# ToyotaResearchInstitute/conex

Measured on AMD Instinct MI355X. Metric: Newton KKT-solves/sec (assemble+factor+solve), 1000x(20x20) PSD blocks, fp64, higher is better.
Workload: dtype f64

## Files before the change

conex_amd/csrc/kkt_context.hip:

```cpp
#include <hip/hip_ext.h>
#include "kkt_internal.h"
#include "kernels_cone.hip.h"
#include "kernels_gemm.hip.h"
#include "kernels_kkt_big.hip.h"
#include "kernels_oct.hip.h"
#include "kernels_lmi.hip.h"
#include "lmi_fused_mfma.h"
#include "kernels_lmi_sparse.hip.h"
#include "kernels_lmi_rows.hip.h"
#include "kernels_lmi_large.hip.h"
#include "kernels_quad.hip.h"


namespace cxk_host {

int Fail(cxk_context* ctx, const char* msg) {
  ctx->err = msg;
  fprintf(stderr, "conex_kkt_hip: %s\n", msg);
  return CXK_FAILURE;
}

bool IsUnique(int N, int m, const int* x) {
  std::vector<char> seen(N > 0 ? N : 1, 0);
  for (int i = 0; i < m; i++) {
// ... 879 lines not shown
    const size_t lds = sizeof(double) * 65 * ((NA_) > (NB_) ? (NA_) : (NB_)) + sizeof(SnRec) * (size_t)std::min(nchain, kChainRing); \
    if (mode == 0)                                                                                          \
      tree_chain_lean<0, NA_, SA_, NB_, SB_><<<1, 64, lds, ctx->stream>>>(                                  \
          ctx->plan, ctx->p_rec.p, pos0, nchain, ctx->slab.p, ctx->y.p, ctx->d_fail.p, RhsIn{});            \
    else                                                                                                    \
      tree_chain_lean<1, NA_, SA_, NB_, SB_><<<1, 64, lds, ctx->stream>>>(                                  \
          ctx->plan, ctx->p_rec.p, pos0, nchain, ctx->slab.p, ctx->y.p, ctx->d_fail.p, ctx->rhs_in);        \
  }
    CXK_CHAIN(8, 8, 8, 8)
    CXK_CHAIN(16, 8, 16, 8)
    CXK_CHAIN(24, 0, 24, 0)
    CXK_CHAIN(24, 8, 24, 8)
    CXK_CHAIN(32, 16, 32, 16)
    CXK_CHAIN(8, 8, 24, 0)
    CXK_CHAIN(16, 8, 24, 0)
    CXK_CHAIN(8, 8, 16, 8)
    CXK_CHAIN(24, 0, 24, 8)
    CXK_CHAIN(24, 0, 32, 16)
#undef CXK_CHAIN
    CXK_DEMAND(done, "internal error: no tree_chain_lean instance for the chain's shapes");
    CXK_TRY(hipGetLastError());
  return CXK_SUCCESS;
}

int MakeFusedTreeArgs(cxk_context* ctx, FusedTreeArgs* out) {
  if (*ctx->fx_flag != 0.0) {
    CXK_TRY(hipStreamSynchronize(ctx->stream));
    CXK_TRY(hipMemcpy(ctx->fx_hand.p, ctx->fx_hand_init.data(), sizeof(double) * ctx->fx_hand_init.size(), hipMemcpyHostToDevice));
    unsigned long long bits = kFusedSentinel;
    double sent;
    memcpy(&sent, &bits, sizeof(sent));
    std::vector<double> ys(ctx->fx_ysig.n, sent);
    CXK_TRY(hipMemcpy(ctx->fx_ysig.p, ys.data(), sizeof(double) * ys.size(), hipMemcpyHostToDevice));
    if (ctx->fx_done.p) {
      CXK_TRY(hipMemset(ctx->fx_done.p, 0, sizeof(unsigned long long) * ctx->fx_done.n));
      ctx->fx_done_target = 0;
    }
    *ctx->fx_flag = 0.0;
    ctx->timeout_pending = true;
  }
  FusedTreeArgs& a = *out;
  a.rec = ctx->fx_rec.p;
  a.count = (int)ctx->level_sn.size();
  a.G = ctx->G.p;
  a.AWc = ctx->AWc.p;
  a.AQcc = ctx->AQcc.p;
  a.b = ctx->b.p;
  a.AW = ctx->AW.p;
  a.AQc = ctx->AQc.p;
  a.slab = ctx->slab.p;
  a.y = ctx->y.p;
  a.pub = ctx->fx_pub.p;
  a.tg_reg = ctx->tg_reg.p;
  a.xreg = ctx->fx_xreg.p;
  a.xsrc = ctx->fx_xsrc.p;
  a.rsrc = ctx->fx_rsrc.p;
  a.hand = ctx->fx_hand.p;
  a.hand_stride = (long long)(ctx->fx_hand.n / 2);
  a.updb_base = ctx->fx_updb_base;
  a.ysig = ctx->fx_ysig.p;
  a.ysig_stride = (long long)(ctx->fx_ysig.n / 2);
  a.gen = (int)(ctx->fused_gen++ & 1u);
  a.tgen = (int)(ctx->fused_tgen & 1u);
  a.fwd_stride = ctx->fx_fwd_stride;
  a.y_stride = ctx->md.N;
  a.y3 = ctx->y3.p;
  a.fail = ctx->d_fail.p;
  a.tag = ctx->fail_tag;
  a.k = a.bs = a.cs = a.cb = a.cq = a.cw = 0;
  a.k_from = nullptr;
  a.comb = 0;
  a.form = 0;
  a.sc = ctx->sc.p;
  a.sys_sc = ctx->sys_sc.p;
  a.K = (int)ctx->cons.size();
  a.host_flag = ctx->fx_flag;
  a.up_sleep = 30;
  a.count_up = ctx->fused_shard ? ctx->fused_up : a.count;
  a.x = ctx->xbuf.p;
  a.n_xs = ctx->n_xs;
  a.n_xv = ctx->n_xv;
  a.xg = ctx->fx_xg.p;
  a.as_src = ctx->as_src.p;
  a.xs_pt = ctx->xs_pt.p;
  a.pt_ptr = ctx->pt_ptr.p;
  a.pt_src = ctx->pt_src.p;
  a.xr = ctx->fx_xr.p;
  a.rs_src = ctx->rs_src.p;
  a.pf_ptr = ctx->pf_ptr.p;
  a.pf_src = ctx->pf_src.p;
  a.done = ctx->fx_done.p;
  a.done_target = 0;
  return CXK_SUCCESS;
}

int ShardAllReduce(cxk_context* ctx, double* buf, size_t count, int op);
// ... 28 lines not shown
  a.done_target = ++ctx->fx_done_target;
  const bool hook = ctx->debug_timeout_at >= 0 && ctx->fused_launches++ == ctx->debug_timeout_at;
  CXK_TRY(LaunchFusedTree(a, ctx->fused_sa, ctx->fused_sb, kFusedShardUp, ctx->stream));
  if (hook && ctx->debug_timeout_site == CXK_DEBUG_FUSED_SHARD_UP && DebugReportTimeout(ctx)) return CXK_FAILURE;
  if (*ctx->fx_flag != 0.0) {
    static const double kTimedOut[2] = {1.0, 1.0};
    CXK_TRY(hipMemcpyAsync(ctx->xbuf.p + ExchangeCount(ctx) - 2, kTimedOut, sizeof(kTimedOut), hipMemcpyHostToDevice,
                           ctx->stream));
  }
  if (ShardAllReduce(ctx, ctx->xbuf.p, (size_t)ExchangeCount(ctx), 0 )) return CXK_FAILURE;
  ctx->shard_fused_tag = ctx->asm_tag;
  ctx->shard_launch_collectives = ctx->collectives;
  CXK_TRY(LaunchFusedTree(a, ctx->fused_sa, ctx->fused_sb, kFusedShardTop, ctx->stream));
  if (hook && ctx->debug_timeout_site == CXK_DEBUG_FUSED_SHARD_TOP && DebugReportTimeout(ctx)) return CXK_FAILURE;
  return CXK_SUCCESS;
}

int LaunchFusedTreeSolve(cxk_context* ctx) {
  const cxk_context::AsmPending ap = ctx->asm_pending;
  ctx->asm_pending.on = false;
  FusedTreeArgs a;
  if (MakeFusedTreeArgs(ctx, &a)) return CXK_FAILURE;
  ctx->asm_tag = ctx->asm_tag >= (1 << 30) ? 1 : ctx->asm_tag + 1;
  a.tag = ctx->fail_tag = ctx->asm_tag;
  a.k = ap.k;
  a.bs = ap.bs;
  a.cs = ap.cs;
  a.cb = ap.cb;
  a.cq = ap.cq;
  a.cw = ap.cw;
  a.comb = ap.with_rhs == 2;
  if (ap.with_rhs == 3) {
    ctx->fused_tgen++;
    CXK_TRY(LaunchFusedTree(a, ctx->fused_sa, ctx->fused_sb, kFusedTriple, ctx->stream, ctx->clk_e0, ctx->clk_e1));
  } else if (ctx->fused_split) {
    CXK_TRY(LaunchFusedTree(a, ctx->fused_sa, ctx->fused_sb, kFusedUp, ctx->stream));
    CXK_TRY(LaunchFusedTree(a, ctx->fused_sa, ctx->fused_sb, kFusedDown, ctx->stream));
  } else {
    CXK_TRY(LaunchFusedTree(a, ctx->fused_sa, ctx->fused_sb, kFusedFull, ctx->stream, ctx->clk_e0, ctx->clk_e1));
  }
  if (ctx->debug_timeout_at >= 0 && ctx->fused_launches++ == ctx->debug_timeout_at &&
      ctx->debug_timeout_site == CXK_DEBUG_FUSED_FACTOR && DebugReportTimeout(ctx))
    return CXK_FAILURE;
  return CXK_SUCCESS;
}

int LaunchFusedTreeSweep(cxk_context* ctx) {
  FusedTreeArgs a;
  if (MakeFusedTreeArgs(ctx, &a)) return CXK_FAILURE;
  const RhsIn& ri = ctx->rhs_in;
  a.form = ri.form;
  a.k = ri.k;
  a.k_from = ri.k_from;
  a.bs = ri.bs;
  a.cs = ri.cs;
  a.cb = ri.cb;
  a.cq = ri.cq;
  a.cw = ri.cw;
  if (ctx->fused_split) {
    CXK_TRY(LaunchFusedTree(a, ctx->fused_sa, ctx->fused_sb, kFusedForward, ctx->stream));
    CXK_TRY(LaunchFusedTree(a, ctx->fused_sa, ctx->fused_sb, kFusedDown, ctx->stream));
  } else {
    CXK_TRY(LaunchFusedTree(a, ctx->fused_sa, ctx->fused_sb, kFusedSolve, ctx->stream, ctx->clk_e0, ctx->clk_e1));
  }
  return CXK_SUCCESS;
}

bool FusedTimedOut(const cxk_context* ctx) { return ctx->timeout_pending || (ctx->fx_flag && *ctx->fx_flag != 0.0); }

int DisableFusedTree(cxk_context* ctx) {
  CXK_TRY(hipStreamSynchronize(ctx->stream));
// ... 2350 lines not shown
```

conex_amd/csrc/kkt_internal.h:

```cpp
#pragma once
#include <hip/hip_runtime.h>
#include <dlfcn.h>
#include <rccl/rccl.h>

#include <algorithm>
#include <atomic>
#include <cfloat>
#include <climits>
#include <cmath>
#include <cstdio>
#include <cstdlib>
#include <cstring>
#include <iterator>
#include <map>
#include <memory>
#include <string>
#include <tuple>
#include <vector>

#include "../../include/conex_kkt_hip.h"
#include "kernels_kkt.hip.h"
#include "kernels_kkt_top.hip.h"
#include "lmi_types.h"
#include "symbolic.h"
// ... 157 lines not shown
  DevBuf<SnRec> p_rec;
  DevBuf<int> pub_dst, pubb_dst;
  DevBuf<double> upd, updb, xbuf;
  DevBuf<int64_t> xs_off, pt_dst, pt_src;
  DevBuf<int> xv_idx, pt_ptr, pf_ptr, pf_src, xs_pt;
  int64_t as_T = 0;
  bool fused_asm = false;
  DevBuf<AsmRec> asm_rec;
  DevBuf<GatherRec> as_rec2;
  DevBuf<ResidRec> rs_rec2;
  DevBuf<int> rs_var2;
  int64_t as_T2 = 0;
  int rs_N2 = 0;
  struct AsmPending {
    bool on = false;
    int with_rhs = 0;
    double k = 0, bs = 0, cs = 0, cb = 0, cq = 0, cw = 0;
  } asm_pending;
  bool fused_tree = false;
  bool fused_split = false;
  bool fused_sweep = false;
  bool fused_shard = false;
  int fused_up = 0;
  DevBuf<GatherRec> fx_xg;
  DevBuf<ResidRec> fx_xr;
  DevBuf<unsigned long long> fx_done;
  unsigned long long fx_done_target = 0;
  int fused_sa = 0, fused_sb = 0;
  DevBuf<int> fx_rec, fx_xreg;
  DevBuf<long long> fx_xsrc, fx_rsrc;
  DevBuf<int> fx_pub;
  DevBuf<double> fx_hand, fx_ysig;
  std::vector<double> fx_hand_init;
  long long fx_updb_base = 0;
  long long fx_fwd_stride = 0;
  unsigned fused_tgen = 0;
  DevBuf<double> y3;
  bool y3_valid = false;
  double y3_bs = 0, y3_cs = 0;
  bool y_deferred = false;
  bool no_y_deferral = false;
  DevBuf<unsigned long long> y_done;
  unsigned long long y_done_target = 0;
  bool no_triple = false;
  unsigned fused_gen = 0;
  double* fx_flag = nullptr;
  int debug_timeout_at = -1, debug_timeout_site = 0, fused_launches = 0;
  int fused_timeouts = 0;
  bool timeout_pending = false;
  bool timeout_unreported = false;
  long long shard_settled_seq = -1;
  int shard_fused_tag = 0;
  long long collectives = 0, shard_launch_collectives = 0;
  bool debug_stream_ordered = false;
  long long calls = 0, redo_call = -1;
  bool asm_deferred = false;
  bool forward_all_lean = false;
  RhsIn rhs_in{};
  int asm_tag = 0;
  bool fail_clean = false;
  int fail_tag = 0;
  FactorPlan plan{};
  unsigned long long lanczos_calls = 0;
  int dual_start = -1;
  bool use_ldlt = false;
  DevBuf<int> d_tr, d_reg;
// ... 84 lines not shown
```

conex_amd/csrc/kkt_plans.hip:

```cpp
#define CXK_DEVICE_FUNCTIONS_ONLY
#include "kkt_internal.h"
#include "big_chol.h"

namespace cxk_host {

void ComputeTreeStructure(cxk_context* ctx) {
  const Layout& L = ctx->lay;
  const int K = ctx->md.K;
  ctx->t_ns.assign(K, 0);
  ctx->t_nsep.assign(K, 0);
  ctx->t_start.assign(K, 0);
  ctx->t_level.assign(K, 0);
  ctx->t_parent.assign(K, -1);
  for (int e = 0; e < K; e++) {
    ctx->t_ns[e] = L.supernode_size[e];
    ctx->t_nsep[e] = (int)L.separators[e].size();
    ctx->t_start[e] = L.supernode_start[e];
    if (ctx->t_nsep[e] > 0) ctx->t_parent[e] = L.var_to_sn[L.separators[e][0]];
  }
  for (int i = 0; i < K; i++) {
    if (ctx->t_ns[i] == 0) continue;
    for (int v : L.separators[i]) {
      const int p = L.var_to_sn[v];
      if (ctx->t_level[p] < ctx->t_level[i] + 1) ctx->t_level[p] = ctx->t_level[i] + 1;
    }
  }
  ctx->nlev = 0;
  for (int e = 0; e < K; e++)
    if (ctx->t_ns[e] > 0) ctx->nlev = std::max(ctx->nlev, ctx->t_level[e] + 1);
}

double ConstraintWork(const ConstraintRec& c) {
  const double n = c.n, m = c.m;
// ... 84 lines not shown
      ctx->sn_mine[e] = 1;
      ctx->owned[i] = (rr++ % G) == ctx->rank;
    } else {
      const bool mine = owner_of_root[root_of[e]] == ctx->rank;
      ctx->sn_mine[e] = mine;
      ctx->owned[i] = mine;
    }
  }
  for (int p = 0; p < ctx->md.N; p++) ctx->var_valid[p] = ctx->sn_mine[ctx->lay.var_to_sn[p]];
  for (int e = 0; e < K; e++)
    if (ctx->sn_top[e]) {
      const int64_t n = ctx->t_ns[e];
      ctx->n_xs += n * (n + 1) / 2 + n * ctx->t_nsep[e];
      ctx->n_xv += (int)n;
    }
}

namespace {

struct PlanSwitches {
  bool no_big_dataflow = getenv("CXK_NO_BIG_DATAFLOW") != nullptr;
  bool debug_levels = getenv("CXK_DEBUG_LEVELS") != nullptr;
  bool no_lean = getenv("CXK_NO_LEAN") != nullptr;
  bool no_ranges = getenv("CXK_NO_RANGES") != nullptr;
  bool keep_top = getenv("CXK_KEEP_TOP") != nullptr;
  bool no_chain = getenv("CXK_NO_CHAIN") != nullptr;
  bool no_back_pairs = getenv("CXK_NO_BACK_PAIRS") != nullptr;
  bool no_fused_asm = getenv("CXK_NO_FUSED_ASM") != nullptr;
  bool no_fused_shard = getenv("CXK_NO_FUSED_SHARD") != nullptr;
  bool no_fused_tree = getenv("CXK_NO_FUSED_TREE") != nullptr;
  bool no_fused_wide = getenv("CXK_NO_FUSED_WIDE") != nullptr;
  bool fused_split = getenv("CXK_FUSED_SPLIT") != nullptr;
  bool fused_level_order = getenv("CXK_FUSED_LEVEL_ORDER") != nullptr;
  bool no_fused_sweep = getenv("CXK_NO_FUSED_SWEEP") != nullptr;
  bool no_top_dense = getenv("CXK_NO_TOP_DENSE") != nullptr;
};

struct Verdict {
  bool ok = true;
  const char* why = nullptr;
  bool check(bool cond, const char* msg) {
    ok = ok && cond;
    if (!ok && !why) why = msg;
    return ok;
  }
  void note(const char* msg) { check(true, msg); }
  int refuse(const PlanSwitches& sw, const char* strategy) const {
    if (sw.debug_levels) fprintf(stderr, "%s not taken: %s\n", strategy, why ? why : "(unnamed check)");
    return CXK_SUCCESS;
  }
};

template <typename Rec>
std::vector<Rec> Flatten(const std::vector<std::vector<int64_t>>& lists, std::vector<int>* ptr, std::vector<int64_t>* src) {
  std::vector<Rec> recs(lists.size());
  ptr->assign(lists.size() + 1, 0);
  for (size_t t = 0; t < lists.size(); t++) {
    for (int64_t q : lists[t]) src->push_back(q);
    (*ptr)[t + 1] = (int)src->size();
    const int len = (*ptr)[t + 1] - (*ptr)[t];
    recs[t].first = len > 0 ? (*src)[(*ptr)[t]] : -1;
    recs[t].beg = (*ptr)[t] + 1;
    recs[t].extra = len > 0 ? len - 1 : 0;
  }
  return recs;
}
// ... 695 lines not shown
      ok = rg.per[pvar].size() == 1 && rg.per[pvar][0] == ar.r_off + r[a];
      var_own[pvar] = 1;
    }
  }
  v.check(ok, "a level-0 supernode that is not a leaf with single sources in its own constraint's block");
  if (!v.ok) return v.refuse(sw, "fused assembly");
  std::vector<GatherRec> g2;
  for (size_t t = 0; t < ag.rec.size(); t++)
    if (!slab_own[t]) g2.push_back(ag.rec[t]);
  std::vector<ResidRec> r2;
  std::vector<int> v2;
  for (int pvar = 0; pvar < N; pvar++)
    if (!var_own[pvar]) {
      r2.push_back(rg.rec[pvar]);
      v2.push_back(pvar);
    }
  ctx->as_T2 = (int64_t)g2.size();
  ctx->rs_N2 = (int)v2.size();
  if (g2.empty()) g2.push_back(GatherRec{0, -1, 0, 0});
  if (v2.empty()) {
    r2.push_back(ResidRec{-1, 0, 0});
    v2.push_back(0);
  }
  CXK_TRY(ctx->asm_rec.upload(arecs));
  CXK_TRY(ctx->as_rec2.upload(g2));
  CXK_TRY(ctx->rs_rec2.upload(r2));
  CXK_TRY(ctx->rs_var2.upload(v2));
  ctx->fused_asm = true;
  return CXK_SUCCESS;
}


struct FusedTables {
  std::vector<int> recs, xreg, pub;
  std::vector<long long> xsrc, rsrc;
};

bool FusedTreeShapes(const cxk_context* ctx, const PlanSwitches& sw, const UpdateSlots& u, Verdict& v, int* sa, int* sb) {
  const int nlev = ctx->nlev;
  const std::vector<int>& ns = ctx->t_ns;
  const int cnt_all = (int)ctx->level_sn.size();
  const bool wide_single = v.ok && ctx->world <= 1 && cnt_all == 1 && ctx->md.K >= 1 && ns[ctx->level_sn[0]] > 32 &&
                           ns[ctx->level_sn[0]] <= 64 && ctx->t_nsep[ctx->level_sn[0]] == 0 && !sw.no_fused_wide;
  if (wide_single) {
    *sa = *sb = ((ns[ctx->level_sn[0]] + 7) / 8 * 8) << 8;
    return true;
  }
  std::vector<int> shapes;
  for (int l = 0; l < nlev && v.ok; l++) {
    if (ctx->level_ptr[l + 1] == ctx->level_ptr[l]) continue;
    v.ok = !ctx->level_big[l] && ctx->level_nh[l] == ctx->level_ptr[l + 1] - ctx->level_ptr[l];
    for (auto& sg : ctx->level_segs[l]) {
      v.ok = v.ok && sg.shape != 0 && sg.inl;
      if (std::find(shapes.begin(), shapes.end(), sg.shape) == shapes.end()) shapes.push_back(sg.shape);
    }
    for (int pos = ctx->level_ptr[l]; pos < ctx->level_ptr[l + 1] && v.ok; pos++) {
      const int e = ctx->level_sn[pos];
      v.ok = u.tg_ptr[e + 1] - u.tg_ptr[e] <= kFastTargets && u.m[e] <= kFusedMaxSlots && u.mf[e] <= kFusedMaxSlots;
    }
  }
  for (size_t i = 0; i < shapes.size(); i++)
    if ((shapes[i] & 255) == 0)
      for (size_t j = 0; j < shapes.size(); j++)
        if (j != i && shapes[i] >= 0 && (shapes[j] >> 8) == (shapes[i] >> 8) && (shapes[j] & 255) > 0) {
          shapes[i] = -1;
          break;
        }
// ... 105 lines not shown
    w[62] = (int)(xbase >> 32);
    w[63] = ctx->t_level[e];
    for (auto& xe : extra) {
      ft->xreg.push_back(xe.first);
      for (size_t q2 = 0; q2 < mx; q2++) ft->xsrc.push_back(q2 < xe.second.size() ? (long long)xe.second[q2] : -1ll);
    }
    if (mr > 0)
      for (int a = 0; a < nse; a++) {
        const auto& lst = rg.per[start[e] + a];
        for (size_t q2 = 0; q2 < mr; q2++) ft->rsrc.push_back(lst.size() > 1 && q2 < lst.size() ? (long long)lst[q2] : -1ll);
      }
    v.ok = ft->rsrc.size() < (size_t)INT32_MAX && ft->xreg.size() < (size_t)INT32_MAX;
  }
}

void FusedTreePublished(const cxk_context* ctx, const UpdateSlots& u, const std::vector<int>& pos_of, size_t n_upd,
                        size_t n_updb, Verdict& v, FusedTables* ft) {
  const Layout& L = ctx->lay;
  const int cnt_all = (int)ctx->level_sn.size();
  for (int pos = 0; pos < cnt_all && v.ok; pos++) {
    const int e = ctx->level_sn[pos];
    for (int x : L.separators[e]) v.check(pos_of[L.var_to_sn[x]] > pos, "a consumer at a lower position");
  }
  v.ok = v.ok && n_upd + n_updb + 8 < (size_t)INT32_MAX;
  for (int pos = 0; pos < cnt_all && v.ok; pos++) {
    const int e = ctx->level_sn[pos];
    const int nsep = ctx->t_nsep[e];
    int* w = ft->recs.data() + (size_t)pos * kFusedRecWords;
    w[21] = w[22] = 0;
    w[23] = (int)ft->pub.size();
    for (int64_t t = 0; t < (int64_t)nsep * (nsep + 1) / 2; t++) ft->pub.push_back(u.pub_dst[(size_t)(u.upd_off[e] + t)]);
    for (int c = 0; c < nsep; c++) ft->pub.push_back((int)n_upd + u.pubb_dst[(size_t)(u.updb_off[e] + c)]);
  }
}

void DealOverXcds(const cxk_context* ctx, const std::vector<int>& pos_of, std::vector<int>* recs) {
  const Layout& L = ctx->lay;
  const int cnt_all = (int)ctx->level_sn.size();
  std::vector<std::vector<int>> kids(cnt_all);
  std::vector<int> roots;
  for (int pos = 0; pos < cnt_all; pos++) {
    int par = INT32_MAX;
    for (int v : L.separators[ctx->level_sn[pos]]) par = std::min(par, pos_of[L.var_to_sn[v]]);
    if (par == INT32_MAX)
      roots.push_back(pos);
    else
      kids[par].push_back(pos);
  }
  std::vector<int> dfs, stack(roots.rbegin(), roots.rend());
  dfs.reserve(cnt_all);
  while (!stack.empty()) {
    const int u = stack.back();
    stack.pop_back();
    dfs.push_back(u);
    for (auto it = kids[u].rbegin(); it != kids[u].rend(); ++it) stack.push_back(*it);
  }
  if ((int)dfs.size() != cnt_all) return;
  std::vector<int> perm(cnt_all, -1);
  size_t at = 0;
  for (int x = 0; x < 8; x++) {
    const int n = (cnt_all - x + 7) / 8;
    std::vector<int> mine(dfs.begin() + at, dfs.begin() + at + n);
    at += n;
    std::sort(mine.begin(), mine.end());
    for (int i = 0; i < n; i++) perm[8 * i + x] = mine[i];
  }
// ... 27 lines not shown
  const size_t us = (size_t)u.slots + 1 + kPullPad, ubs = (size_t)u.slotsb + 2 + kPullPad;
  std::vector<int> pos_of(ctx->md.K, -1);
  for (int pos = 0; pos < cnt_all; pos++) pos_of[ctx->level_sn[pos]] = pos;
  if (v.ok) FusedTreePublished(ctx, u, pos_of, us, ubs, v, &ft);
  bool split = false;
  if (v.ok) {
    const int occ = FusedTreeOccupancy(sa, sb, sharded);
    v.check(occ >= 2, "occupancy query failed");
    split = (int64_t)cnt_all + 1 > (int64_t)(occ - 1) * ctx->cus || sw.fused_split;
    if (sharded) {
      v.check((int64_t)(cnt_all - cnt_up) + 1 <= (int64_t)(occ - 1) * ctx->cus,
              "the replicated top exceeds the resident wavefronts");
      split = false;
    }
  }
  if (v.ok && sharded) {
    std::vector<GatherRec> xg(x.xs.size() + 1, GatherRec{0, -1, 0, 0});
    for (size_t t = 0; t < x.xs.size() && v.ok; t++) {
      const int et = ag.entry_of[x.xs[t]];
      v.ok = et >= 0;
      if (v.ok) xg[t] = ag.rec[et];
    }
    v.note("a top entry without a gather record");
    std::vector<ResidRec> xr(x.xv.size() + 1, ResidRec{-1, 0, 0});
    for (size_t j = 0; j < x.xv.size(); j++) xr[j] = rg.rec[x.xv[j]];
    if (v.ok) {
      CXK_TRY(ctx->fx_xg.upload(xg));
      CXK_TRY(ctx->fx_xr.upload(xr));
      CXK_TRY(ctx->fx_done.alloc(64 * 16, true));
      ctx->fx_done_target = 0;
    }
  }
  if (!v.ok) return v.refuse(sw, "whole-tree launch");
  ft.xreg.resize(ft.xreg.size() + kPullPad, 0);
  ft.xsrc.resize(ft.xsrc.size() + kPullPad * kFusedExtraMax, -1ll);
  ft.rsrc.resize(ft.rsrc.size() + 64 * kFusedExtraMax, -1ll);
  ft.pub.resize(ft.pub.size() + 64, (int)u.slots);
  const double sent = [] {
    double d;
    const unsigned long long bits = kFusedSentinel;
    memcpy(&d, &bits, sizeof(d));
    return d;
  }();
  const size_t hs = us + 3 * ubs + 8;
  ctx->fx_updb_base = (long long)us;
  ctx->fx_fwd_stride = (long long)ubs;
  ctx->fx_hand_init.assign(2 * hs, 0.0);
  for (size_t t = 0; t + 64 < ft.pub.size(); t++) {
    const int d = ft.pub[t];
    if (d != (int)u.slots && d != (int)us + u.slotsb) {
      ctx->fx_hand_init[d] = ctx->fx_hand_init[hs + d] = sent;
      if ((size_t)d >= us)
        for (size_t q = 1; q < 3; q++) ctx->fx_hand_init[d + q * ubs] = ctx->fx_hand_init[hs + d + q * ubs] = sent;
    }
  }
  if (!split && !sharded && !sw.fused_level_order) DealOverXcds(ctx, pos_of, &ft.recs);
  CXK_TRY(ctx->fx_rec.upload(ft.recs));
  CXK_TRY(ctx->fx_xreg.upload(ft.xreg));
  CXK_TRY(ctx->fx_xsrc.upload(ft.xsrc));
  CXK_TRY(ctx->fx_rsrc.upload(ft.rsrc));
  CXK_TRY(ctx->fx_pub.upload(ft.pub));
  CXK_TRY(ctx->fx_hand.upload(ctx->fx_hand_init));
  CXK_TRY(ctx->fx_ysig.upload(std::vector<double>(6 * (size_t)N, sent)));
  CXK_TRY(ctx->y3.alloc(3 * (size_t)N, true));
  ctx->fused_tgen = 0;
  ctx->y3_valid = false;
  if (!ctx->fx_flag) {
    CXK_TRY(hipHostMalloc(reinterpret_cast<void**>(&ctx->fx_flag), 64, hipHostMallocDefault));
    *ctx->fx_flag = 0.0;
  }
  ctx->fused_sa = sa;
  ctx->fused_sb = sb;
  ctx->fused_gen = 0;
  ctx->fused_tree = true;
  ctx->fused_split = split;
  ctx->fused_shard = sharded;
  ctx->fused_up = cnt_up;
  ctx->fused_sweep = !sharded && !sw.no_fused_sweep;
  if (sw.debug_levels)
    fprintf(stderr, "whole tree in %s: %d supernodes, shapes <%d,%d> <%d,%d>, %zu entries / %zu variables with further sources\n",
            sharded ? "two launches around the exchange (own subtrees up + pack, top + down)" : split ? "two launches (up, down)" : "one launch", cnt_all, sa >> 8, sa & 255, sb >> 8, sb & 255,
            ft.xreg.size() - kPullPad, ft.rsrc.size());
  return CXK_SUCCESS;
}

int PlanTopDense(cxk_context* ctx, const PlanSwitches& sw, const UpdateSlots& u) {
  const Layout& L = ctx->lay;
  const int K = ctx->md.K, N = ctx->md.N, nlev = ctx->nlev;
  const std::vector<int>& ns = ctx->t_ns;
  const std::vector<int>& nsep = ctx->t_nsep;
  const std::vector<int>& start = ctx->t_start;
  ctx->top_dense.on = false;
  ctx->dense_level = nlev;
  Verdict v;
  v.check(ctx->world <= 1 && !ctx->use_ldlt && !sw.no_top_dense, "sharded, LDLT or CXK_NO_TOP_DENSE");
  int dt = -1;
  if (v.ok) {
    int cols = 0, count = 0;
    bool clean = true;
    for (int l = nlev - 1; l >= 0 && clean; l--) {
      if (ctx->level_nh[l] != ctx->level_ptr[l + 1] - ctx->level_ptr[l]) break;
      for (int pos = ctx->level_ptr[l]; pos < ctx->level_ptr[l + 1]; pos++) {
        cols += ns[ctx->level_sn[pos]];
        count++;
      }
      if (cols > kTopMaxCols || count > kTopMaxSn) break;
      if (ctx->level_big[l]) dt = l;
    }
  }
  v.check(dt >= 0, "no level of mid-size supernodes among the top levels that fit");
  std::vector<int> tsn;
  int T = 0;
  if (v.ok) {
    for (int pos = ctx->level_ptr[dt]; pos < ctx->level_ptr[nlev]; pos++) tsn.push_back(ctx->level_sn[pos]);
    std::sort(tsn.begin(), tsn.end());
// ... 229 lines not shown
```

conex_amd/csrc/tree_fused.h:

```cpp
#pragma once
#include <hip/hip_runtime.h>

#include <cstdint>

namespace cxk {

constexpr unsigned long long kFusedSentinel = 0x7FF4C0DEC0DE5EEDull;

constexpr int kFusedRecWords = 64;
constexpr int kFusedExtraTargets = 128;
constexpr int kFusedExtraSlots = 8;
constexpr int kFusedExtraMax = 64;
constexpr int kFusedMaxSlots = 4096;

struct GatherRec;
struct ResidRec;

struct FusedTreeArgs {
  const int* rec;
  int count;
  const double *G, *AWc, *AQcc, *b;
  double *AW, *AQc;
  double* slab;
  double* y;
  const int* pub;
  const int* tg_reg;
  const int* xreg;
  const long long* xsrc;
  const long long* rsrc;
  double* hand;
  long long hand_stride;
  long long updb_base;
  double* ysig;
  long long ysig_stride;
  int gen;
  int tgen;
  long long fwd_stride, y_stride;
  double* y3;
  int* fail;
  int tag;
  double k, bs, cs;
  double cb, cq, cw;
  int comb;
  int form;
  const double* k_from;
  const double* sc;
  double* sys_sc;
  int K;
  double* host_flag;
  int up_sleep;
  int count_up;
  double* x;
  long long n_xs;
  int n_xv;
  const GatherRec* xg;
  const int64_t* as_src;
  const int* xs_pt;
  const int* pt_ptr;
  const int64_t* pt_src;
  const ResidRec* xr;
  const int64_t* rs_src;
  const int* pf_ptr;
  const int* pf_src;
  unsigned long long* done;
  unsigned long long done_target;
};

constexpr int FusedRhsLane(int nsmax, int smax) { return (nsmax == 16 && smax == 8) || (nsmax == 24 && smax == 0) ? 24 : -1; }

enum FusedTreeMode { kFusedFull = 0, kFusedSolve = 1, kFusedUp = 2, kFusedForward = 3, kFusedDown = 4,
                     kFusedShardUp = 5, kFusedShardTop = 6, kFusedTriple = 7 };
// ... 8 lines not shown
```

conex_amd/csrc/tree_fused.hip:

```cpp
#include <hip/hip_runtime.h>
#include <hip/hip_ext.h>

#include <type_traits>

#define CXK_DEVICE_FUNCTIONS_ONLY
#include "kernels_kkt.hip.h"
#include "kernels_kkt_top.hip.h"
#include "tree_fused.h"

namespace cxk {

constexpr int kFusedSpinLimit = 1 << 18;

#ifdef CXK_FUSED_STAMPS
constexpr int kFusedStampWaves = 8192;
__device__ long long g_fused_tree_stamp[kFusedStampWaves * 16];
#define FT_STAMP(i) ft_stamp[i] = __builtin_amdgcn_s_memrealtime()
#define FT_COUNT(i, v) ft_stamp[i] = (v)
#define FT_STAMP_DECL long long ft_stamp[16] = {0, 0, 0, 0, 0, 0, 0, 0, 0, 0, 0, 0, 0, 0, 0, 0}
#define FT_STAMP_FLUSH(level)                                                              \
  do {                                                                                     \
    if ((threadIdx.x & 63) == 0 && blockIdx.x < kFusedStampWaves) {                        \
      ft_stamp[15] = (level);                                                              \
      for (int i_ = 0; i_ < 16; i_++) g_fused_tree_stamp[blockIdx.x * 16 + i_] = ft_stamp[i_]; \
// ... 489 lines not shown
      for (int c = 0; c < SMAX; c++) my[(SMAX + NRHS) * lane + c] = a[NSMAX + c];
#pragma unroll
      for (int q = 0; q < NCOL; q++) my[(SMAX + NRHS) * lane + SMAX + q] = a[RB + q];
      WaveSync();
#pragma unroll
      for (int r = 0; r < PR; r++) {
        const double v = -my[prd[r]];
        if (lane + 64 * r < nv) StoreAgent((NRHS > 1 && pdt[r] ? handT : handG) + pd[r], v);
      }
      WaveSync();
    }
  }
  FT_STAMP(7);
  if constexpr (UP_ONLY) {
#pragma unroll
    for (int j = 0; j < NSMAX; j++)
      if (j < lim) base[o0 + j * st] = a[j];
    if (is_row) {
      A.y[R.start + lane] = a[NCOL > 0 ? RB : 0];
      A.AW[R.start + lane] = awv;
      A.AQc[R.start + lane] = aqv;
    }
    if constexpr (SMAX > 0) {
      if (s > 0) {
#pragma unroll
        for (int r = 0; r < PR; r++)
          if (lane + 64 * r < nv) StoreAgent(handO + pd[r], SentinelValue());
      }
    }
    return;
  }
  const int cnt = R.bs_end - R.bs_beg;
  const bool active = is_row;
  if constexpr (NSMAX <= 32) {
#pragma unroll
    for (int j = 0; j < NSMAX; j++) my[65 * j + lane] = a[j];
  }
  WaveSync();
  if (cnt > 0) {
#pragma unroll
    for (int j = 0; j < NSMAX; j++)
      if (j < lim) base[o0 + j * st] = a[j];
  }
  FT_STAMP(8);
  const int li = active ? lane : 0;
  double col[NSMAX];
#pragma unroll
  for (int k = 0; k < NSMAX; k++) col[k] = my[65 * li + k];
  double dg = my[66 * li];
  FT_STAMP(9);
  constexpr int QN = SMAX < 8 ? SMAX : 8;
  double bv[QN > 0 ? QN : 1], yv[QN > 0 ? QN : 1], Mb[QN > 0 ? QN : 1];
  double yvx[NRHS > 1 ? NRHS - 1 : 1][QN > 0 ? QN : 1];
  bv[0] = Mb[0] = 0.0;
#pragma unroll
  for (int qq = 0; qq < (QN > 0 ? QN : 1); qq++) {
    yv[qq] = 0.0;
#pragma unroll
    for (int q = 0; q < (NRHS > 1 ? NRHS - 1 : 1); q++) yvx[q][qq] = 0.0;
  }
  if constexpr (QN > 0) {
#pragma unroll
    for (int qq = 0; qq < QN; qq++) {
      const unsigned sw = qq < cnt ? (unsigned)R.sep[qq] : 0u;
      bv[qq] = my[65 * li + NSMAX + (int)(sw >> 26)];
    }
// ... 8 lines not shown
#pragma unroll
    for (int q = 0; q < NRHS - 1; q++) ubx[q] = active ? my[65 * li + RL + 1 + q] : 0.0;
  } else {
    ub = active ? a[NCOL > 0 ? RB : 0] : 0.0;
#pragma unroll
    for (int q = 0; q < NCOL - 1; q++) ubx[q] = active ? a[RB + 1 + q] : 0.0;
  }
  if constexpr (QN > 0) {
#pragma unroll
    for (int qq = 0; qq < QN; qq++) Mb[qq] = (qq < cnt && active) ? bv[qq] : 0.0;
  }
  {
    const double dinv = 1.0 / dg;
#pragma unroll
    for (int k = NSMAX - 1; k >= 0; k--) {
      if (lane == k) ub *= dinv;
      ub = fma(-col[k], ReadLane(ub, k), ub);
      if constexpr (NRHS > 1) {
#pragma unroll
        for (int q = 0; q < NRHS - 1; q++) {
          if (lane == k) ubx[q] *= dinv;
          ubx[q] = fma(-col[k], ReadLane(ubx[q], k), ubx[q]);
        }
      }
      if constexpr (QN > 0) {
        if (cnt > 0) {
#pragma unroll
          for (int qq = 0; qq < QN; qq++) {
            if (lane == k) Mb[qq] *= dinv;
            Mb[qq] = fma(-col[k], ReadLane(Mb[qq], k), Mb[qq]);
          }
        }
      }
    }
  }
  constexpr bool ROW0 = NSMAX <= 16 && QN > 0;
  double vsep = 0.0, vsepx[NRHS > 1 ? NRHS - 1 : 1];
#pragma unroll
  for (int q = 0; q < (NRHS > 1 ? NRHS - 1 : 1); q++) vsepx[q] = 0.0;
  if constexpr (ROW0) {
#pragma unroll
    for (int qq = 0; qq < QN; qq++) {
      Mb[qq] = -Mb[qq];
      asm volatile("" : "+v"(Mb[qq]));
    }
  }
  if constexpr (QN > 0) {
    if (cnt > 0) {
      const int sepw = __builtin_amdgcn_ds_bpermute(4 * (24 + (lane < 8 ? lane : 0)), w);
      const int sidx = lane < cnt ? (sepw & 0x3ffffff) : (R.sep[0] & 0x3ffffff);
      const double* src = ysG + sidx;
      double v;
      double vx[NRHS > 1 ? NRHS - 1 : 1];
      vx[0] = 0.0;
      for (int spin = 0;; spin++) {
        v = LoadAgent(src);
        bool pending = (lane < cnt) & IsSentinel(v);
        if constexpr (NRHS > 1) {
#pragma unroll
          for (int q = 0; q < NRHS - 1; q++) {
            vx[q] = LoadAgent(ysT + (int64_t)(1 + q) * A.y_stride + sidx);
            pending |= (lane < cnt) & IsSentinel(vx[q]);
          }
        }
        if (__ballot(pending) == 0) {
          FT_COUNT(14, spin);
          break;
        }
        if (spin >= kFusedSpinLimit) {
          ReportTimeout(A);
          break;
        }
        __builtin_amdgcn_s_sleep(1);
      }
      v = lane < cnt ? v : 0.0;
      if constexpr (NRHS > 1) {
#pragma unroll
        for (int q = 0; q < NRHS - 1; q++) vx[q] = lane < cnt ? vx[q] : 0.0;
      }
      if constexpr (ROW0) {
        vsep = v;
        if constexpr (NRHS > 1) {
#pragma unroll
          for (int q = 0; q < NRHS - 1; q++) vsepx[q] = vx[q];
        }
      } else {
#pragma unroll
        for (int qq = 0; qq < QN; qq++) yv[qq] = ReadLane(v, qq);
        if constexpr (NRHS > 1) {
#pragma unroll
          for (int q = 0; q < NRHS - 1; q++)
#pragma unroll
            for (int qq = 0; qq < QN; qq++) yvx[q][qq] = ReadLane(vx[q], qq);
        }
      }
    }
  }
  FT_STAMP(5);
  double accx[NRHS > 1 ? NRHS - 1 : 1];
  accx[0] = 0.0;
  double acc = ub;
  if constexpr (ROW0) {
    if constexpr (NRHS > 1) {
      static_assert(NRHS == 3, "two further right-hand sides");
      accx[0] = ubx[0];
      accx[1] = ubx[1];
// ... 7 lines not shown
      if constexpr (qq < QN) {
        FmacRowBcast<qq>(acc, vsep, Mb[qq]);
        if constexpr (NRHS > 1) {
          FmacRowBcast<qq>(accx[0], vsepx[0], Mb[qq]);
          FmacRowBcast<qq>(accx[1], vsepx[1], Mb[qq]);
        }
        self(self, std::integral_constant<int, qq + 1>{});
      }
    };
    chain(chain, std::integral_constant<int, 0>{});
  } else {
    if constexpr (NRHS > 1 && QN > 0) {
#pragma unroll
      for (int q = 0; q < NRHS - 1; q++) {
        accx[q] = ubx[q];
#pragma unroll
        for (int qq = 0; qq < QN; qq++) accx[q] = fma(-Mb[qq], yvx[q][qq], accx[q]);
      }
    } else if constexpr (NRHS > 1) {
#pragma unroll
      for (int q = 0; q < NRHS - 1; q++) accx[q] = ubx[q];
    }
    if constexpr (QN > 0) {
#pragma unroll
      for (int qq = 0; qq < QN; qq++) acc = fma(-Mb[qq], yv[qq], acc);
    }
  }
  if (active) StoreAgent(ysG + R.start + lane, acc);
  if constexpr (NRHS > 1) {
#pragma unroll
    for (int q = 0; q < NRHS - 1; q++)
      if (active) StoreAgent(ysT + (int64_t)(1 + q) * A.y_stride + R.start + lane, accx[q]);
  }
  FT_STAMP(6);
  if constexpr (ROWRHS) {
    if (__ballot(active && !(acc == acc)) != 0 && lane == 0) atomicExch(A.fail + 1, A.tag);
  }
  if (active) {
    if constexpr (NRHS == 3) {
      A.y3[R.start + lane] = acc;
      A.y3[A.y_stride + R.start + lane] = accx[0];
      A.y3[2 * A.y_stride + R.start + lane] = accx[1];
      A.y[R.start + lane] = accx[0] - acc;
      StoreAgent(ysTO + A.y_stride + R.start + lane, SentinelValue());
      StoreAgent(ysTO + 2 * A.y_stride + R.start + lane, SentinelValue());
    } else {
      A.y[R.start + lane] = acc;
    }
    A.AW[R.start + lane] = awv;
    A.AQc[R.start + lane] = aqv;
    StoreAgent(ysO + R.start + lane, SentinelValue());
  }
  if (NSMAX <= 32 && cnt == 0) {
#pragma unroll
    for (int j = 0; j < NSMAX; j++)
      if (j < lim) base[o0 + j * st] = a[j];
  }
  if constexpr (SMAX > 0) {
    if (s > 0) {
#pragma unroll
      for (int r = 0; r < PR; r++)
        if (lane + 64 * r < nv) StoreAgent((NRHS > 1 && pdt[r] ? handTO : handO) + pd[r], SentinelValue());
    }
  }
  FT_STAMP_FLUSH(f(31));
}

template <int NSMAX, int SMAX, int PHASE = 0>
__device__ __forceinline__ void FusedSolveSupernode(const FusedTreeArgs& A, const int w) {
  static_assert(NSMAX + SMAX <= 64, "one lane per panel row");
  constexpr int MFMAX = kFastSlots;
  constexpr int NVMAX = SMAX * (SMAX + 1) / 2 + SMAX;
  constexpr int PR = (NVMAX + 63) / 64;
  const int lane = threadIdx.x & 63;
  const SnRec R = DecodeRec(w);
  const int ns = R.ns, s = R.nsep;
  const bool is_row = lane < ns;
  const int sc = lane - NSMAX;
  const bool is_sep = sc >= 0 && sc < s;
  const double* base = A.slab + R.diag_off;
  const unsigned rel = (unsigned)(R.offd_off - R.diag_off);
  const unsigned o0 = is_row ? (unsigned)lane : (is_sep ? rel + (unsigned)(sc * ns) : 0u);
  const unsigned st = is_row ? (unsigned)ns : 1u;
  const int lim = is_row ? lane : (is_sep ? ns : 0);
  const int gen = A.gen;
  double* handG = A.hand + (int64_t)gen * A.hand_stride;
  double* handO = A.hand + (int64_t)(gen ^ 1) * A.hand_stride;
  double* ysG = A.ysig + (int64_t)gen * A.ysig_stride;
  double* ysO = A.ysig + (int64_t)(gen ^ 1) * A.ysig_stride;
// ... 431 lines not shown
```

Measured before the change: 23080.

## Add multi-level jump closures to fused tree back-solve to shorten dependency chains

```diff
diff --git a/conex_amd/csrc/kkt_context.hip b/conex_amd/csrc/kkt_context.hip
--- a/conex_amd/csrc/kkt_context.hip
+++ b/conex_amd/csrc/kkt_context.hip
@@ -935,6 +935,11 @@
     memcpy(&sent, &bits, sizeof(sent));
     std::vector<double> ys(ctx->fx_ysig.n, sent);
     CXK_TRY(hipMemcpy(ctx->fx_ysig.p, ys.data(), sizeof(double) * ys.size(), hipMemcpyHostToDevice));
+    for (DevBuf<double>* jb : {&ctx->fx_jrows, &ctx->fx_yrep})
+      if (jb->n > 0) {
+        ys.assign(jb->n, sent);
+        CXK_TRY(hipMemcpy(jb->p, ys.data(), sizeof(double) * ys.size(), hipMemcpyHostToDevice));
+      }
     if (ctx->fx_done.p) {
       CXK_TRY(hipMemset(ctx->fx_done.p, 0, sizeof(unsigned long long) * ctx->fx_done.n));
       ctx->fx_done_target = 0;
@@ -965,6 +970,10 @@
   a.ysig_stride = (long long)(ctx->fx_ysig.n / 2);
   a.gen = (int)(ctx->fused_gen++ & 1u);
   a.tgen = (int)(ctx->fused_tgen & 1u);
+  a.jgen = (int)(ctx->fused_jgen & 1u);
+  a.jlist = ctx->fx_jlist.p;
+  a.jrows = ctx->fx_jrows.p;
+  a.yrep = ctx->fx_yrep.p;
   a.fwd_stride = ctx->fx_fwd_stride;
   a.y_stride = ctx->md.N;
   a.y3 = ctx->y3.p;
@@ -1059,11 +1068,13 @@
   a.comb = ap.with_rhs == 2;
   if (ap.with_rhs == 3) {
     ctx->fused_tgen++;
+    ctx->fused_jgen++;
     CXK_TRY(LaunchFusedTree(a, ctx->fused_sa, ctx->fused_sb, kFusedTriple, ctx->stream, ctx->clk_e0, ctx->clk_e1));
   } else if (ctx->fused_split) {
     CXK_TRY(LaunchFusedTree(a, ctx->fused_sa, ctx->fused_sb, kFusedUp, ctx->stream));
     CXK_TRY(LaunchFusedTree(a, ctx->fused_sa, ctx->fused_sb, kFusedDown, ctx->stream));
   } else {
+    ctx->fused_jgen++;
     CXK_TRY(LaunchFusedTree(a, ctx->fused_sa, ctx->fused_sb, kFusedFull, ctx->stream, ctx->clk_e0, ctx->clk_e1));
   }
   if (ctx->debug_timeout_at >= 0 && ctx->fused_launches++ == ctx->debug_timeout_at &&
diff --git a/conex_amd/csrc/kkt_internal.h b/conex_amd/csrc/kkt_internal.h
--- a/conex_amd/csrc/kkt_internal.h
+++ b/conex_amd/csrc/kkt_internal.h
@@ -213,6 +213,9 @@
   DevBuf<int> fx_pub;
   DevBuf<double> fx_hand, fx_ysig;
   std::vector<double> fx_hand_init;
+  DevBuf<int> fx_jlist;
+  DevBuf<double> fx_jrows, fx_yrep;
+  unsigned fused_jgen = 0;
   long long fx_updb_base = 0;
   long long fx_fwd_stride = 0;
   unsigned fused_tgen = 0;
diff --git a/conex_amd/csrc/kkt_plans.hip b/conex_amd/csrc/kkt_plans.hip
--- a/conex_amd/csrc/kkt_plans.hip
+++ b/conex_amd/csrc/kkt_plans.hip
@@ -1,4 +1,7 @@
 #define CXK_DEVICE_FUNCTIONS_ONLY
+#include <map>
+#include <set>
+
 #include "kkt_internal.h"
 #include "big_chol.h"
 
@@ -149,6 +152,7 @@
   bool no_fused_wide = getenv("CXK_NO_FUSED_WIDE") != nullptr;
   bool fused_split = getenv("CXK_FUSED_SPLIT") != nullptr;
   bool fused_level_order = getenv("CXK_FUSED_LEVEL_ORDER") != nullptr;
+  bool fused_no_jump = getenv("CXK_FUSED_NO_JUMP") != nullptr;
   bool no_fused_sweep = getenv("CXK_NO_FUSED_SWEEP") != nullptr;
   bool no_top_dense = getenv("CXK_NO_TOP_DENSE") != nullptr;
 };
@@ -910,7 +914,7 @@
 
 
 struct FusedTables {
-  std::vector<int> recs, xreg, pub;
+  std::vector<int> recs, xreg, pub, jlist;
   std::vector<long long> xsrc, rsrc;
 };
 
@@ -1082,6 +1086,91 @@
     for (int64_t t = 0; t < (int64_t)nsep * (nsep + 1) / 2; t++) ft->pub.push_back(u.pub_dst[(size_t)(u.upd_off[e] + t)]);
     for (int c = 0; c < nsep; c++) ft->pub.push_back((int)n_upd + u.pubb_dst[(size_t)(u.updb_off[e] + c)]);
   }
+}
+
+int FusedTreeJumps(const cxk_context* ctx, const std::vector<int>& pos_of, FusedTables* ft) {
+  const Layout& L = ctx->lay;
+  const int cnt_all = (int)ctx->level_sn.size();
+  auto rec = [&](int pos) { return ft->recs.data() + (size_t)pos * kFusedRecWords; };
+  auto sep_of = [&](int e) {
+    const int* w = rec(pos_of[e]);
+    std::vector<int> sv;
+    if (w[20] == w[7] - w[6])
+      for (int q = 0; q < w[20]; q++) sv.push_back(w[24 + q] & 0x3ffffff);
+    return sv;
+  };
+  int with = 0;
+  for (int pos = 0; pos < cnt_all; pos++) {
+    const int e = ctx->level_sn[pos];
+    const std::vector<int> own = sep_of(e);
+    if (own.empty()) continue;
+    std::map<int, int> dist;
+    for (int a = ctx->t_parent[e], d = 1; a >= 0 && d <= cnt_all; a = ctx->t_parent[a], d++) dist[a] = d;
+    for (int jump = kFusedJump; jump >= 2; jump--) {
+      std::vector<int> polled, work(own.rbegin(), own.rend());
+      std::map<int, std::vector<int>> rows;
+      std::set<int> seen;
+      bool ok = true;
+      while (!work.empty() && ok) {
+        const int x = work.back();
+        work.pop_back();
+        if (!seen.insert(x).second) continue;
+        const int a = L.var_to_sn[x];
+        const auto it = dist.find(a);
+        ok = it != dist.end();
+        const std::vector<int> as = ok ? sep_of(a) : std::vector<int>();
+        if (ok && it->second < jump && !as.empty()) {
+          rows[a].push_back(x);
+          for (int y : as) work.push_back(y);
+        } else {
+          polled.push_back(x);
+        }
+      }
+      if (!ok || rows.empty()) break;
+      size_t nrows = 0;
+      for (auto& r : rows) nrows += r.second.size();
+      if (polled.size() + nrows > 64) continue;
+      std::sort(polled.begin(), polled.end());
+      std::vector<int> groups;
+      for (auto& r : rows) {
+        std::sort(r.second.begin(), r.second.end());
+        groups.push_back(r.first);
+      }
+      std::sort(groups.begin(), groups.end(), [&](int a, int b) { return dist[a] > dist[b]; });
+      std::map<int, int> lane_of;
+      std::vector<int> lst = {(int)polled.size(), (int)nrows, (int)groups.size(), 0};
+      for (int x : polled) {
+        lane_of[x] = (int)lst.size() - 4;
+        lst.push_back(x);
+      }
+      for (int a : groups) {
+        const int ca = (int)sep_of(a).size();
+        for (int x : rows[a]) {
+          lane_of[x] = (int)lst.size() - 4;
+          lst.push_back(x | ca << 26);
+        }
+      }
+      for (int a : groups) {
+        lst.push_back(lane_of[rows[a][0]]);
+        lst.push_back((int)rows[a].size());
+        const std::vector<int> as = sep_of(a);
+        lst.push_back((int)as.size());
+        for (int y : as) lst.push_back(lane_of.at(y));
+      }
+      lst[3] = (int)lst.size();
+      for (int y : own) lst.push_back(lane_of.at(y));
+      if (lst.size() > (size_t)kFusedJumpList) continue;
+      int* w = rec(pos);
+      w[21] = (int)ft->jlist.size();
+      w[22] |= (int)lst.size();
+      ft->jlist.insert(ft->jlist.end(), lst.begin(), lst.end());
+      for (int a : groups) rec(pos_of[a])[22] |= 1 << 16;
+      for (int x : polled) rec(pos_of[L.var_to_sn[x]])[22] |= 1 << 17;
+      with++;
+      break;
+    }
+  }
+  return with;
 }
 
 void DealOverXcds(const cxk_context* ctx, const std::vector<int>& pos_of, std::vector<int>* recs) {
@@ -1175,6 +1264,7 @@
     }
   }
   if (!v.ok) return v.refuse(sw, "whole-tree launch");
+  const int jumps = !split && !sharded && !sw.fused_no_jump ? FusedTreeJumps(ctx, pos_of, &ft) : 0;
   ft.xreg.resize(ft.xreg.size() + kPullPad, 0);
   ft.xsrc.resize(ft.xsrc.size() + kPullPad * kFusedExtraMax, -1ll);
   ft.rsrc.resize(ft.rsrc.size() + 64 * kFusedExtraMax, -1ll);
@@ -1205,6 +1295,11 @@
   CXK_TRY(ctx->fx_pub.upload(ft.pub));
   CXK_TRY(ctx->fx_hand.upload(ctx->fx_hand_init));
   CXK_TRY(ctx->fx_ysig.upload(std::vector<double>(6 * (size_t)N, sent)));
+  ft.jlist.resize(ft.jlist.size() + kFusedJumpList, 0);
+  CXK_TRY(ctx->fx_jlist.upload(ft.jlist));
+  CXK_TRY(ctx->fx_jrows.upload(std::vector<double>(jumps ? 2 * kFusedJumpPlanes * (size_t)N : 0, sent)));
+  CXK_TRY(ctx->fx_yrep.upload(std::vector<double>(jumps ? 6 * kFusedReplicas * (size_t)N : 0, sent)));
+  ctx->fused_jgen = 0;
   CXK_TRY(ctx->y3.alloc(3 * (size_t)N, true));
   ctx->fused_tgen = 0;
   ctx->y3_valid = false;
@@ -1221,9 +1316,9 @@
   ctx->fused_up = cnt_up;
   ctx->fused_sweep = !sharded && !sw.no_fused_sweep;
   if (sw.debug_levels)
-    fprintf(stderr, "whole tree in %s: %d supernodes, shapes <%d,%d> <%d,%d>, %zu entries / %zu variables with further sources\n",
+    fprintf(stderr, "whole tree in %s: %d supernodes, shapes <%d,%d> <%d,%d>, %zu entries / %zu variables with further sources, %d closures\n",
             sharded ? "two launches around the exchange (own subtrees up + pack, top + down)" : split ? "two launches (up, down)" : "one launch", cnt_all, sa >> 8, sa & 255, sb >> 8, sb & 255,
-            ft.xreg.size() - kPullPad, ft.rsrc.size());
+            ft.xreg.size() - kPullPad, ft.rsrc.size(), jumps);
   return CXK_SUCCESS;
 }
 
diff --git a/conex_amd/csrc/tree_fused.h b/conex_amd/csrc/tree_fused.h
--- a/conex_amd/csrc/tree_fused.h
+++ b/conex_amd/csrc/tree_fused.h
@@ -12,6 +12,10 @@
 constexpr int kFusedExtraSlots = 8;
 constexpr int kFusedExtraMax = 64;
 constexpr int kFusedMaxSlots = 4096;
+constexpr int kFusedJump = 4;
+constexpr int kFusedJumpList = 128;
+constexpr int kFusedJumpPlanes = 11;
+constexpr int kFusedReplicas = 8;
 
 struct GatherRec;
 struct ResidRec;
@@ -37,6 +41,10 @@
   int tgen;
   long long fwd_stride, y_stride;
   double* y3;
+  const int* jlist;
+  double* jrows;
+  double* yrep;
+  int jgen;
   int* fail;
   int tag;
   double k, bs, cs;
diff --git a/conex_amd/csrc/tree_fused.hip b/conex_amd/csrc/tree_fused.hip
--- a/conex_amd/csrc/tree_fused.hip
+++ b/conex_amd/csrc/tree_fused.hip
@@ -545,6 +545,29 @@
   }
   const int cnt = R.bs_end - R.bs_beg;
   const bool active = is_row;
+  constexpr bool JUMPS = !UP_ONLY && !FROM_X;
+  const int jw = JUMPS ? __builtin_amdgcn_readlane(w, 22) : 0;
+  const int jlen = jw & 0xffff;
+  const bool jpub = (jw >> 16) & 1, janc = (jw >> 17) & 1;
+  const int64_t jN = A.y_stride;
+  double* jrJ = A.jrows + (int64_t)A.jgen * kFusedJumpPlanes * jN;
+  double* jrT = A.jrows + (int64_t)A.tgen * kFusedJumpPlanes * jN;
+  int jlw0 = 0, jlw1 = 0, jlab = 0, jol = 0;
+  if (JUMPS && jlen > 0) {
+    const int* jl = A.jlist + __builtin_amdgcn_readlane(w, 21);
+    jlw0 = jl[lane];
+    jlw1 = jl[64 + lane];
+    jlab = jl[4 + lane];
+    jol = jl[__builtin_amdgcn_readlane(jlw0, 3) + (lane < cnt ? lane : 0)];
+  }
+  constexpr int JRR = (kFusedReplicas * NSMAX + 63) / 64;
+  int jrep[JRR], jrow[JRR];
+#pragma unroll
+  for (int r2 = 0; r2 < JRR; r2++) {
+    const int t = lane + 64 * r2, nsd = ns > 0 ? ns : 1;
+    jrep[r2] = janc ? t / nsd : kFusedReplicas;
+    jrow[r2] = janc ? t - (t / nsd) * nsd : 0;
+  }
   if constexpr (NSMAX <= 32) {
 #pragma unroll
     for (int j = 0; j < NSMAX; j++) my[65 * j + lane] = a[j];
@@ -619,6 +642,17 @@
           }
         }
       }
+    }
+  }
+  if constexpr (JUMPS && QN > 0) {
+    if (jpub && active) {
+      const int64_t p = R.start + lane;
+      StoreAgent(jrJ + p, ub);
+#pragma unroll
+      for (int q = 0; q < NRHS - 1; q++) StoreAgent(jrT + (1 + q) * jN + p, ubx[q]);
+#pragma unroll
+      for (int qq = 0; qq < QN; qq++)
+        if (qq < cnt) StoreAgent(jrJ + (3 + qq) * jN + p, Mb[qq]);
     }
   }
   constexpr bool ROW0 = NSMAX <= 16 && QN > 0;
@@ -640,25 +674,133 @@
       double v;
       double vx[NRHS > 1 ? NRHS - 1 : 1];
       vx[0] = 0.0;
-      for (int spin = 0;; spin++) {
-        v = LoadAgent(src);
-        bool pending = (lane < cnt) & IsSentinel(v);
-        if constexpr (NRHS > 1) {
+      if (JUMPS && jlen > 0) {
+        auto jword = [&](int i) { return i < 64 ? __builtin_amdgcn_readlane(jlw0, i) : __builtin_amdgcn_readlane(jlw1, i - 64); };
+        const int npoll = jword(0), nl = npoll + jword(1), ngroups = jword(2);
+        const bool is_poll = lane < npoll, is_jrow = lane >= npoll && lane < nl;
+        const int jp = is_poll || is_jrow ? (jlab & 0x3ffffff) : 0, jmc = is_jrow ? (int)((unsigned)jlab >> 26) : 0;
+        int opl[8], mygrp = -1;
+#pragma unroll
+        for (int qq = 0; qq < 8; qq++) opl[qq] = 0;
+        {
+          int at = 4 + nl;
+          for (int g = 0; g < ngroups; g++) {
+            const int lb = jword(at), nr = jword(at + 1), cg = jword(at + 2);
+            at += 3;
+            const bool mine = lane >= lb && lane < lb + nr;
+            mygrp = mine ? g : mygrp;
+#pragma unroll
+            for (int qq = 0; qq < 8; qq++)
+              if (qq < cg) opl[qq] = mine ? jword(at + qq) : opl[qq];
+            at += cg;
+          }
+        }
+        const double* jfirst = jrJ + __builtin_amdgcn_readlane(jp, npoll);
+        int spin = 0;
+        for (;; spin++) {
+          if (!IsSentinel(LoadAgent(jfirst))) break;
+          if (spin >= kFusedSpinLimit) {
+            ReportTimeout(A);
+            break;
+          }
+          SleepUnits(16);
+        }
+        double ju0, jux[NRHS > 1 ? NRHS - 1 : 1], jm[8];
+        jux[0] = 0.0;
+        for (;; spin++) {
+          ju0 = LoadAgent(jrJ + jp);
+          bool pending = is_jrow & IsSentinel(ju0);
 #pragma unroll
           for (int q = 0; q < NRHS - 1; q++) {
-            vx[q] = LoadAgent(ysT + (int64_t)(1 + q) * A.y_stride + sidx);
-            pending |= (lane < cnt) & IsSentinel(vx[q]);
-          }
-        }
-        if (__ballot(pending) == 0) {
-          FT_COUNT(14, spin);
-          break;
-        }
-        if (spin >= kFusedSpinLimit) {
-          ReportTimeout(A);
-          break;
-        }
-        __builtin_amdgcn_s_sleep(1);
+            jux[q] = LoadAgent(jrT + (1 + q) * jN + jp);
+            pending |= is_jrow & IsSentinel(jux[q]);
+          }
+#pragma unroll
+          for (int qq = 0; qq < 8; qq++) {
+            jm[qq] = LoadAgent(jrJ + (qq < jmc ? 3 + qq : 0) * jN + jp);
+            pending |= is_jrow & (qq < jmc) & IsSentinel(jm[qq]);
+          }
+          if (__ballot(pending) == 0) break;
+          if (spin >= kFusedSpinLimit) {
+            ReportTimeout(A);
+            break;
+          }
+          __builtin_amdgcn_s_sleep(1);
+        }
+        const int rp = (int)(blockIdx.x & (kFusedReplicas - 1));
+        const double* ya = A.yrep + (int64_t)(rp * 2 + A.jgen) * 3 * jN + jp;
+        const double* yt = A.yrep + (int64_t)(rp * 2 + A.tgen) * 3 * jN + jp;
+        double yl, ylx[NRHS > 1 ? NRHS - 1 : 1];
+        ylx[0] = 0.0;
+        for (spin = 0;; spin++) {
+          yl = LoadAgent(ya);
+          bool pending = is_poll & IsSentinel(yl);
+#pragma unroll
+          for (int q = 0; q < NRHS - 1; q++) {
+            ylx[q] = LoadAgent(yt + (1 + q) * jN);
+            pending |= is_poll & IsSentinel(ylx[q]);
+          }
+          if (__ballot(pending) == 0) {
+            FT_COUNT(14, spin);
+            break;
+          }
+          if (spin >= kFusedSpinLimit) {
+            ReportTimeout(A);
+            break;
+          }
+          __builtin_amdgcn_s_sleep(1);
+        }
+        FT_STAMP(13);
+        yl = is_poll ? yl : 0.0;
+#pragma unroll
+        for (int q = 0; q < NRHS - 1; q++) ylx[q] = is_poll ? ylx[q] : 0.0;
+        for (int g = 0; g < ngroups; g++) {
+          double acc0 = ju0, accq[NRHS > 1 ? NRHS - 1 : 1];
+          accq[0] = 0.0;
+#pragma unroll
+          for (int q = 0; q < NRHS - 1; q++) accq[q] = jux[q];
+          double yo[8];
+#pragma unroll
+          for (int qq = 0; qq < 8; qq++) yo[qq] = __shfl(yl, opl[qq]);
+#pragma unroll
+          for (int qq = 0; qq < 8; qq++) acc0 = qq < jmc ? fma(-jm[qq], yo[qq], acc0) : acc0;
+#pragma unroll
+          for (int q = 0; q < NRHS - 1; q++) {
+#pragma unroll
+            for (int qq = 0; qq < 8; qq++) yo[qq] = __shfl(ylx[q], opl[qq]);
+#pragma unroll
+            for (int qq = 0; qq < 8; qq++) accq[q] = qq < jmc ? fma(-jm[qq], yo[qq], accq[q]) : accq[q];
+          }
+          const bool mine = mygrp == g;
+          yl = mine ? acc0 : yl;
+#pragma unroll
+          for (int q = 0; q < NRHS - 1; q++) ylx[q] = mine ? accq[q] : ylx[q];
+        }
+        v = __shfl(yl, jol);
+#pragma unroll
+        for (int q = 0; q < NRHS - 1; q++) vx[q] = __shfl(ylx[q], jol);
+      } else {
+        for (int spin = 0;; spin++) {
+          v = LoadAgent(src);
+          bool pending = (lane < cnt) & IsSentinel(v);
+          if constexpr (NRHS > 1) {
+#pragma unroll
+            for (int q = 0; q < NRHS - 1; q++) {
+              vx[q] = LoadAgent(ysT + (int64_t)(1 + q) * A.y_stride + sidx);
+              pending |= (lane < cnt) & IsSentinel(vx[q]);
+            }
+          }
+          if (__ballot(pending) == 0) {
+            FT_COUNT(14, spin);
+            break;
+          }
+          if (spin >= kFusedSpinLimit) {
+            ReportTimeout(A);
+            break;
+          }
+          __builtin_amdgcn_s_sleep(1);
+        }
+        FT_STAMP(13);
       }
       v = lane < cnt ? v : 0.0;
       if constexpr (NRHS > 1) {
@@ -732,6 +874,19 @@
     for (int q = 0; q < NRHS - 1; q++)
       if (active) StoreAgent(ysT + (int64_t)(1 + q) * A.y_stride + R.start + lane, accx[q]);
   }
+  if (JUMPS && janc) {
+#pragma unroll
+    for (int r2 = 0; r2 < JRR; r2++) {
+      const double val = __shfl(acc, jrow[r2]);
+      if (jrep[r2] < kFusedReplicas) StoreAgent(A.yrep + (int64_t)(jrep[r2] * 2 + A.jgen) * 3 * jN + R.start + jrow[r2], val);
+#pragma unroll
+      for (int q = 0; q < NRHS - 1; q++) {
+        const double vq = __shfl(accx[q], jrow[r2]);
+        if (jrep[r2] < kFusedReplicas)
+          StoreAgent(A.yrep + ((int64_t)(jrep[r2] * 2 + A.tgen) * 3 + 1 + q) * jN + R.start + jrow[r2], vq);
+      }
+    }
+  }
   FT_STAMP(6);
   if constexpr (ROWRHS) {
     if (__ballot(active && !(acc == acc)) != 0 && lane == 0) atomicExch(A.fail + 1, A.tag);
@@ -755,6 +910,27 @@
 #pragma unroll
     for (int j = 0; j < NSMAX; j++)
       if (j < lim) base[o0 + j * st] = a[j];
+  }
+  if (JUMPS && jpub && active) {
+    double* jrJO = A.jrows + (int64_t)(A.jgen ^ 1) * kFusedJumpPlanes * jN + R.start + lane;
+    double* jrTO = A.jrows + (int64_t)(A.tgen ^ 1) * kFusedJumpPlanes * jN + R.start + lane;
+    StoreAgent(jrJO, SentinelValue());
+#pragma unroll
+    for (int q = 0; q < NRHS - 1; q++) StoreAgent(jrTO + (1 + q) * jN, SentinelValue());
+#pragma unroll
+    for (int qq = 0; qq < 8; qq++)
+      if (qq < cnt) StoreAgent(jrJO + (3 + qq) * jN, SentinelValue());
+  }
+  if (JUMPS && janc) {
+#pragma unroll
+    for (int r2 = 0; r2 < JRR; r2++)
+      if (jrep[r2] < kFusedReplicas) {
+        const int64_t o = R.start + jrow[r2];
+        StoreAgent(A.yrep + (int64_t)(jrep[r2] * 2 + (A.jgen ^ 1)) * 3 * jN + o, SentinelValue());
+#pragma unroll
+        for (int q = 0; q < NRHS - 1; q++)
+          StoreAgent(A.yrep + ((int64_t)(jrep[r2] * 2 + (A.tgen ^ 1)) * 3 + 1 + q) * jN + o, SentinelValue());
+      }
   }
   if constexpr (SMAX > 0) {
     if (s > 0) {
```

After: 23010, median of 3. Within noise of the previous version (-0.3%).
